# yamiel-abreu/distributed-pytorch-training

Measured on AMD Instinct MI355X. Metric: images/sec (whole node) ResNet-50 bf16 training, higher is better.
Workload: dtype bf16

## Files before the change

csrc/bindings.cpp:

```cpp
#include <ATen/ATen.h>
#include <c10/hip/HIPGuard.h>
#include <c10/hip/HIPStream.h>
#include <torch/extension.h>

#include "kernels/kernels.h"
#include "host_comm.h"
#include "pg_comm.h"
#include "rccl_comm.h"
#include "watchdog.h"
#include "reducer.h"

namespace py = pybind11;
using at::Tensor;

namespace {

hipStream_t cur_stream(const Tensor& t) {
  return c10::hip::getCurrentHIPStream(t.device().index()).stream();
}

dpt::WireType wire_of(const Tensor& t) {
  switch (t.scalar_type()) {
    case at::kFloat: return dpt::WireType::kF32;
    case at::kBFloat16: return dpt::WireType::kBF16;
// ... 1136 lines not shown
        py::arg("mask_out") = py::none());
  m.def("bn_apply", &bn_apply, py::arg("x"), py::arg("residual"), py::arg("a"), py::arg("b"), py::arg("relu"));
  m.def("bn_apply_aff", &bn_apply_aff, py::arg("x"), py::arg("x2"), py::arg("coef"), py::arg("coef2"),
        py::arg("mask_out") = py::none());
  m.def("bn2_bwd_partials", &bn2_bwd_partials, py::arg("dz"), py::arg("x"), py::arg("x2"), py::arg("weight"),
        py::arg("weight2"), py::arg("mean"), py::arg("invstd"), py::arg("mean2"), py::arg("invstd2"), py::arg("p1"),
        py::arg("p2"), py::arg("p3"), py::arg("want_dparams"));
  m.def("bn_bwd", &bn_bwd, py::arg("grad_output"), py::arg("grad_output2"), py::arg("y"), py::arg("x"),
        py::arg("weight"), py::arg("mean"), py::arg("invstd"), py::arg("relu"), py::arg("want_dz"),
        py::arg("want_dparams"), py::arg("coef") = py::none());
  m.def("ln_supported", &dpt::ln_supported, py::arg("D"));
  m.def("ln_fwd", &ln_fwd, py::arg("x"), py::arg("a"), py::arg("bias"), py::arg("gamma"), py::arg("beta"),
        py::arg("eps"), py::arg("out_kind") = 1);
  m.def("ln_bwd", &ln_bwd, py::arg("grad_s"), py::arg("grad_h"), py::arg("s"), py::arg("mean"), py::arg("rstd"),
        py::arg("gamma"), py::arg("want_ga"), py::arg("bias_like"), py::arg("want_dparams"));
  m.def("gelu_fwd", &gelu_fwd, py::arg("u"), py::arg("bias"));
  m.def("gelu_bwd", &gelu_bwd, py::arg("grad"), py::arg("u"), py::arg("bias"), py::arg("want_dbias"));
  m.def("linear_dgrad_dgelu", &linear_dgrad_dgelu, py::arg("grad"), py::arg("wt"), py::arg("u"), py::arg("bias"));
  m.def("vit_set_gelu_blocks_per_cu", &dpt::vit_set_gelu_blocks_per_cu, py::arg("n"));
  m.def("copy_rows16", &copy_rows16, py::arg("src"), py::arg("dst"));
  m.def("bias_grad16", &bias_grad16, py::arg("grad"), py::arg("out_kind"));
  m.def("sum_partials", &sum_partials, py::arg("part"), py::arg("out_kind"));
  m.def("colsum_rows", &colsum_rows, py::arg("part"), py::arg("out_kind"));
  m.def("maxpool_fwd", &maxpool_fwd, py::arg("x"), py::arg("k"), py::arg("stride"), py::arg("pad"),
        py::arg("bn_coef") = py::none());
  m.def("gap_bwd", &gap_bwd, py::arg("g"), py::arg("H"), py::arg("W"), py::arg("dtype"));
  m.def("gap_bwd_bnr", &gap_bwd_bnr, py::arg("g"), py::arg("y"), py::arg("x"), py::arg("mean"));
  m.def("maxpool_bwd", &maxpool_bwd, py::arg("grad_output"), py::arg("idx"), py::arg("H"), py::arg("W"),
        py::arg("k"), py::arg("stride"), py::arg("pad"), py::arg("grad_output2") = py::none(),
        py::arg("bn_x") = py::none(), py::arg("bn_mean") = py::none(), py::arg("bn_coef") = py::none());
  m.def("conv_fwd", &conv_fwd, py::arg("x"), py::arg("w"), py::arg("stride"), py::arg("pad"), py::arg("want_stats"),
        py::arg("out_h") = 0, py::arg("out_w") = 0);
  m.def("space_to_depth2", &space_to_depth2, py::arg("x"), py::arg("out_f16") = false);
  m.def("conv_wgrad", &conv_wgrad, py::arg("grad_output"), py::arg("x"), py::arg("weight_shape"), py::arg("stride"),
        py::arg("pad"), py::arg("fp32_out"), py::arg("target_blocks") = 0);
  m.def("conv_f32_fwd", &conv_f32_fwd, py::arg("x"), py::arg("w"), py::arg("stride"), py::arg("pad"),
        py::arg("split") = false);
  m.def("conv_f32_dgrad", &conv_f32_dgrad, py::arg("grad_output"), py::arg("w"), py::arg("stride"), py::arg("pad"),
        py::arg("H"), py::arg("W"), py::arg("split") = false);
  m.def("conv_f32_wgrad", &conv_f32_wgrad, py::arg("grad_output"), py::arg("x"), py::arg("weight_shape"),
        py::arg("stride"), py::arg("pad"), py::arg("split") = false);
  m.def("im2col", &im2col, py::arg("x"), py::arg("R"), py::arg("S"), py::arg("stride"), py::arg("pad"), py::arg("Kp"));
  m.def("attn_fwd", &attn_fwd, py::arg("qkv"), py::arg("heads"), py::arg("scale"));
  m.def("attn_set_bwd_split", &dpt::attn_set_bwd_split, py::arg("on"));
  m.def("attn_bwd", &attn_bwd, py::arg("qkv"), py::arg("out"), py::arg("grad_output"), py::arg("lse"),
        py::arg("heads"), py::arg("scale"));
  m.def("conv_set_variant", &dpt::conv_set_variant, py::arg("variant"));
  m.def("bn_set_skip_finalize", &dpt::bn_set_skip_finalize, py::arg("on"),
        "measurement only: skip every BatchNorm finalize launch (wrong values; timing upper bound)");
  m.def("conv_set_splitk_policy", &dpt::conv_set_splitk_policy, py::arg("tiles"), py::arg("eager_tiles"),
        py::arg("eager_min_k"), py::arg("target"), "split-K thresholds (A/B knob; <= 0 keeps a value)");
  m.def("conv_set_big", &dpt::conv_set_big, py::arg("on"));
  m.def("conv_set_halo", &dpt::conv_set_halo, py::arg("on"));
  m.def("conv_set_breg", &dpt::conv_set_breg, py::arg("mode"));
  m.def("conv_set_wgrad_stages", &dpt::conv_set_wgrad_stages, py::arg("mode"));
  m.def("conv_get_breg", &dpt::conv_get_breg);
  m.def("conv_set_streamk", &dpt::conv_set_streamk, py::arg("mode"), py::arg("eff") = 0.0);
  m.def("conv_get_streamk", &dpt::conv_get_streamk);
  m.def("conv_sk_prepare", &dpt::conv_sk_prepare);
  m.def("conv_sk_errors", &dpt::conv_sk_errors);
  m.def("conv_sk_blocks", &dpt::conv_sk_blocks, py::arg("tiles"), py::arg("nk"), py::arg("bn"), py::arg("mode"));
  m.def("conv_set_wgrad_target", &dpt::conv_set_wgrad_target, py::arg("blocks"));
  m.def("conv_set_wgrad_halo", &dpt::conv_set_wgrad_halo, py::arg("mode"));
  m.def("conv_fwd_splits", [](int64_t M, int Cout, int64_t K, bool graph) {
          return dpt::conv_fwd_splits_for(M, Cout, K, graph);
        }, py::arg("M"), py::arg("Cout"), py::arg("K"), py::arg("graph") = false);
  m.def("conv_set_splitk", &dpt::conv_set_splitk, py::arg("mode"));
  m.def("conv_get_splitk", &dpt::conv_get_splitk);
  m.def("conv_set_fwd_shape_policy", &dpt::conv_set_fwd_shape_policy, py::arg("bits"));
  m.def("conv_dgrad", &conv_dgrad, py::arg("grad_output"), py::arg("w"), py::arg("pad"));
  m.def("conv_dgrad_bnstats", &conv_dgrad_bnstats, py::arg("grad_output"), py::arg("w"), py::arg("pad"),
        py::arg("bn_x"), py::arg("bn_mean"), py::arg("bn_coef"), py::arg("bn_y") = py::none(),
        py::arg("bn_res") = py::none(), py::arg("w_flipped") = py::none(), py::arg("bn_x2") = py::none(),
        py::arg("bn_mean2") = py::none(), py::arg("wgrad_reduce") = nullptr, py::arg("bn_mask") = py::none());
  m.def("conv_wt_flip_multi", &conv_wt_flip_multi, py::arg("ws"));
  m.def("conv_dgrad_preflipped", &conv_dgrad_preflipped, py::arg("grad_output"), py::arg("w_flipped"), py::arg("pad"),
        py::arg("wgrad_reduce") = nullptr);
  m.def("bn_bwd_partials", &bn_bwd_partials, py::arg("grad_output"), py::arg("x"), py::arg("weight"), py::arg("mean"),
        py::arg("invstd"), py::arg("coef"), py::arg("p1"), py::arg("p2"), py::arg("want_dparams"),
        py::arg("from_dz") = false);
  m.def("conv_dgrad_s2", &conv_dgrad_s2, py::arg("grad_output"), py::arg("w"), py::arg("pad"), py::arg("H"),
        py::arg("W"), py::arg("bn_x") = py::none(), py::arg("bn_mean") = py::none(), py::arg("bn_coef") = py::none(),
        py::arg("wgrad_reduce") = nullptr);
  m.def("conv_dgrad_flip", &conv_dgrad_flip, py::arg("grad_output"), py::arg("w"), py::arg("pad"),
        py::arg("wgrad_reduce") = nullptr);
  py::class_<PendingReduce, PendingReducePtr>(m, "PendingWgradReduce")
      .def_property_readonly("done", &PendingReduce::done)
      .def_property_readonly("splits", [](const PendingReduce& p) { return p.r.splits; });
  m.def("conv_wgrad_deferred", &conv_wgrad_deferred, py::arg("grad_output"), py::arg("x"), py::arg("weight_shape"),
        py::arg("stride"), py::arg("pad"));
  m.def("conv_reduce_flush", &conv_reduce_flush, py::arg("pending"));
  m.def("rccl_version", []() { return std::string(dpt::rccl_version_string()); });

  py::class_<dpt::Collective, std::shared_ptr<dpt::Collective>>(m, "Collective")
      .def("all_reduce", [](dpt::Collective& c, Tensor t, bool on_current_stream) {
             TORCH_CHECK(t.is_cuda() && t.is_contiguous(), "all_reduce needs a contiguous GPU tensor");
             c10::hip::HIPGuard guard(t.device().index());
             hipStream_t s = cur_stream(t);
             c.all_reduce(t.data_ptr(), (size_t)t.numel(), wire_of(t), on_current_stream ? s : c.stream());
           }, py::arg("tensor"), py::arg("on_current_stream") = true)
      .def("broadcast", [](dpt::Collective& c, Tensor t, int root) {
             TORCH_CHECK(t.is_cuda() && t.is_contiguous(), "broadcast needs a contiguous GPU tensor");
             c10::hip::HIPGuard guard(t.device().index());
             c.broadcast(t.data_ptr(), (size_t)t.numel(), wire_of(t), root, cur_stream(t));
           }, py::arg("tensor"), py::arg("root") = 0)
      .def("abort", &dpt::Collective::abort)
      .def("destroy", &dpt::Collective::destroy)
      .def("check", &dpt::Collective::check)
      .def_property_readonly("kind", &dpt::Collective::kind)
      .def_property_readonly("ops", &dpt::Collective::ops)
      .def_property_readonly("sequence_hash", &dpt::Collective::sequence_hash)
      .def_property_readonly("rank", &dpt::Collective::rank)
      .def_property_readonly("world_size", &dpt::Collective::world_size)
      .def_property_readonly("device", &dpt::Collective::device)
      .def("track", [](dpt::Collective& c) {
             c10::hip::HIPGuard guard(c.device());
             c.track(c10::hip::getCurrentHIPStream(c.device()).stream());
           }, "hand the watchdog a completion marker for the work enqueued on the current stream")
      .def("_test_spin", [](dpt::Collective& c, double ms, bool on_current_stream) {
             TORCH_CHECK(ms >= 0 && ms <= 20000, "spin: 0..20000 ms");
             c10::hip::HIPGuard guard(c.device());
             dpt::launch_spin(ms, on_current_stream ? c10::hip::getCurrentHIPStream(c.device()).stream()
                                                    : c.stream());
           }, py::arg("ms"), py::arg("on_current_stream") = false,
           "test hook: enqueue a wall-clock busy-wait on the communicator (or current) stream");

  py::class_<dpt::RcclComm, dpt::Collective, std::shared_ptr<dpt::RcclComm>>(m, "RcclComm")
      .def(py::init<const std::string&, int, int, int, int, int, double>(), py::arg("unique_id"), py::arg("rank"),
           py::arg("world_size"), py::arg("device"), py::arg("min_ctas") = 0, py::arg("max_ctas") = 0,
           py::arg("init_timeout_s") = 0.0,
           py::call_guard<py::gil_scoped_release>())
      .def_property_readonly("min_ctas", &dpt::RcclComm::min_ctas)
      .def_property_readonly("max_ctas", &dpt::RcclComm::max_ctas)
      .def_property_readonly("handle", &dpt::RcclComm::handle)
      .def("inject_async_error", &dpt::RcclComm::inject_async_error, py::arg("message"))
      .def_static("new_unique_id", []() { return py::bytes(dpt::RcclComm::new_unique_id()); })
      .def("enable_watchdog", &dpt::RcclComm::enable_watchdog, py::arg("timeout_s"), py::arg("poll_s") = 0.5,
           py::arg("exit_grace_s") = 30.0)
      .def_property_readonly("watchdog_tripped", &dpt::RcclComm::watchdog_tripped)
      .def_property_readonly("watchdog_outstanding", &dpt::RcclComm::watchdog_outstanding)
      .def_property_readonly("watchdog_tracked", &dpt::RcclComm::watchdog_tracked)
      .def("async_error", &dpt::RcclComm::async_error);

  py::class_<dpt::HostBridgeComm, dpt::Collective, std::shared_ptr<dpt::HostBridgeComm>>(m, "HostBridgeComm")
      .def(py::init([](py::object ar, py::object bc, int rank, int ws, int dev, bool async_mode, py::object pg) {
             c10::intrusive_ptr<c10d::ProcessGroup> p;
             if (!pg.is_none()) p = pg.cast<c10::intrusive_ptr<c10d::ProcessGroup>>();
             return std::make_shared<dpt::HostBridgeComm>(std::move(ar), std::move(bc), rank, ws, dev, async_mode,
                                                          std::move(p));
           }),
           py::arg("all_reduce_fn"), py::arg("broadcast_fn"), py::arg("rank"), py::arg("world_size"),
           py::arg("device"), py::arg("async_mode") = false, py::arg("process_group") = py::none())
      .def_static("_process_group_size", [](py::object pg) {
             return pg.cast<c10::intrusive_ptr<c10d::ProcessGroup>>()->getSize();
           })
      .def_property_readonly("async_mode", &dpt::HostBridgeComm::async_mode)
      .def_property_readonly("completed", &dpt::HostBridgeComm::completed)
      .def("release_graph_resources", &dpt::HostBridgeComm::release_graph_resources);

  py::class_<dpt::ProcessGroupComm, dpt::Collective, std::shared_ptr<dpt::ProcessGroupComm>>(m, "ProcessGroupComm")
      .def(py::init([](py::object pg, int dev) {
             return std::make_shared<dpt::ProcessGroupComm>(pg.cast<c10::intrusive_ptr<c10d::ProcessGroup>>(), dev);
           }),
           py::arg("process_group"), py::arg("device"))
      .def_property_readonly("backend", &dpt::ProcessGroupComm::backend);

// ... 41 lines not shown
```

csrc/kernels/conv_kernels.hip:

```cpp
#include <algorithm>
#include <cmath>
#include <cstdlib>
#include <mutex>
#include <stdexcept>
#include <type_traits>

#include "carry.h"
#include "gelu.h"
#include "common.h"
#include "kernels.h"
#include "mfma.h"

namespace dpt {


#ifndef DPT_WGRAD_WAVES
#define DPT_WGRAD_WAVES 4
#endif
#ifndef DPT_CONV_HALF_EPI
#define DPT_CONV_HALF_EPI 0
#endif

namespace conv {

constexpr int BM = 128;
constexpr int BK = 64;
constexpr int kThreads = 256;
constexpr int kRowBytes = BK * 2;

__device__ __forceinline__ int swz(int row, int chunk) { return chunk ^ ((row >> 1) & 7); }

__device__ __forceinline__ int opaque_v(int v) {
  asm volatile("" : "+v"(v));
  return v;
}

__device__ __forceinline__ int xcd_remap(int bid, int nwg) {
  const int q = nwg >> 3, r = nwg & 7, xcd = bid & 7, idx = bid >> 3;
  return (xcd < r ? xcd * (q + 1) : r * (q + 1) + (xcd - r) * q) + idx;
}

}

typedef _Float16 f16x8_t __attribute__((ext_vector_type(8)));
typedef _Float16 f16x2_t __attribute__((ext_vector_type(2)));

template <bool F16>
__device__ __forceinline__ f32x16_t cmfma(bf16x8_t a, bf16x8_t b, f32x16_t c) {
  if constexpr (F16)
    return __builtin_amdgcn_mfma_f32_32x32x16_f16(__builtin_bit_cast(f16x8_t, a), __builtin_bit_cast(f16x8_t, b), c,
                                                  0, 0, 0);
  else
    return __builtin_amdgcn_mfma_f32_32x32x16_bf16(a, b, c, 0, 0, 0);
}
template <bool F16>
__device__ __forceinline__ uint32_t cpack(f32x2_t v) {
  if constexpr (F16) return __builtin_bit_cast(uint32_t, __builtin_convertvector(v, f16x2_t));
  else return __builtin_bit_cast(uint32_t, __builtin_convertvector(v, bf16x2_t));
}
template <bool F16>
__device__ __forceinline__ float cunpack(uint32_t u, int h) {
  if constexpr (F16) return (float)__builtin_bit_cast(_Float16, (uint16_t)(h ? (u >> 16) : (u & 0xffffu)));
  else return __uint_as_float(h ? (u & 0xffff0000u) : (u << 16));
}

struct ConvSk {
  float* part = nullptr;
  unsigned* flags = nullptr;
  unsigned* err = nullptr;
  int G = 0;
  uint32_t part_bytes = 0;
};

struct ConvFwdArgs {
  const uint16_t* x = nullptr;
  const uint16_t* w = nullptr;
  uint16_t* y = nullptr;
  float* psum = nullptr;
  float* psq = nullptr;
  int N = 0, H = 0, W = 0, C = 0, Ho = 0, Wo = 0, Cout = 0, R = 0, S = 0, stride = 0, pad = 0;
  int64_t M = 0;
  int m_tiles = 0, n_tiles = 0;
  int mt256 = 0;
  const uint16_t* bnx = nullptr;
  const float* bn_mean = nullptr;
  const float* bn_coef = nullptr;
  float* bp1 = nullptr;
  float* bp2 = nullptr;
  const uint16_t* bny = nullptr;
  const uint16_t* bnres = nullptr;
  const uint8_t* bnmask = nullptr;
  const uint16_t* bias16 = nullptr;
  const uint16_t* bnx2 = nullptr;
  const float* bn_mean2 = nullptr;
  float* bp3 = nullptr;
  int Rw = 0, Sw = 0, tr0 = 0, trs = 0, ts0 = 0, tss = 0;
  int oH = 0, oW = 0, oph = 0, opw = 0;
  int bp_ld = 0, bp_off = 0;
  int f16 = 0;
  float* part = nullptr;
  int splits = 1, kps = 0;
  ReduceCarry red;
  ConvSk sk;
};


template <int N>
__device__ __forceinline__ void vmcnt_wait() {
  asm volatile("s_waitcnt vmcnt(%0)" ::"n"(N) : "memory");
}

template <int RB>
__device__ __forceinline__ bf16x8_t wg_frag(const unsigned char* img, int krow0, int col0, int lane) {
  return tr_frag<RB, false>(img, krow0, col0, lane);
}

__device__ __attribute__((aligned(64))) uint4 g_conv_zero16[4];

template <int BMT, int BN, int STAGES, bool LDSEPI, bool BKN, bool STATS = true, bool BNB = false,
          bool BNR = false, bool REMAP = false, bool ZSIB = false, bool BNR2 = false, bool F16 = false,
          int NT = conv::kThreads, bool SPLIT = false, bool HALO = false, int HB = 1, bool SK = false,
          bool DGELU = false, bool BREG = false>
__global__ __launch_bounds__(NT, (SK || BREG) ? 4 : 2) void conv_fwd_kernel(ConvFwdArgs p) {
  using namespace conv;
  constexpr int BM = BMT;
  constexpr int NW = NT / 64;
  constexpr int WCOL = BREG ? 32 : 64;
  constexpr int WN = BN / WCOL;
  constexpr int WM = NW / WN;
  constexpr int MI = BM / (WM * 32);
  constexpr int NI = WCOL / 32;
  static_assert(WM * WN == NW && MI >= 1 && MI * WM * 32 == BM, "conv_fwd_kernel: bad wave tiling");
  constexpr int A_PER_T = BM * 8 / NT;
  constexpr int B_PER_T = BN * 8 / NT;
  static_assert(!HALO || (BMT == 128 && STAGES == 1 && !BKN && !SPLIT && NT == conv::kThreads), "HALO config");
  static_assert(!SK || (STAGES == 1 && !HALO && !SPLIT && LDSEPI && !BNR2 && NT == conv::kThreads), "SK config");
  static_assert(!DGELU || (BNB && !BNR && !STATS && !REMAP && LDSEPI && !SK), "DGELU config");
  static_assert(!BREG || (BMT == 128 && STAGES == 1 && LDSEPI && !BKN && !SPLIT && !SK && HB == 1 &&
                          NT == conv::kThreads && (BN == 128 || BN == 64)), "BREG config");
  constexpr int HROWS = 136;
  static_assert(HB == 1 || (HALO && HB == 3), "HB");
  constexpr int A_BYTES = (HALO ? HROWS : BM) * kRowBytes, B_BYTES = BN * kRowBytes;
  constexpr int STAGE = A_BYTES + (BREG ? 0 : HB * B_BYTES);
  constexpr int NSTAGE = BREG ? 2 : STAGES;
  constexpr int C_STRIDE = BN * 2 + 16;
  constexpr int RED = 2 * WM * BN * 4;
  constexpr int ZROW = NSTAGE * STAGE;
  constexpr int LDS_MAIN = NSTAGE * STAGE + (HALO ? kRowBytes : 0);
  constexpr bool HALF = DPT_CONV_HALF_EPI && LDSEPI && BM == 128 && NT == conv::kThreads && MI * 32 <= 64 && !BNB &&
                        !SPLIT;
  constexpr int EROWS = HALF ? 64 : BM;
  constexpr int LDS_EPI = (LDSEPI ? EROWS * C_STRIDE : 0) + RED;
  constexpr int LDS = LDS_MAIN > LDS_EPI ? LDS_MAIN : LDS_EPI;
  __shared__ __attribute__((aligned(16))) unsigned char lds[LDS];
  if constexpr (NT == conv::kThreads) {
    if (p.red.blocks) {
      const int nconv = (int)gridDim.x - p.red.blocks;
      if ((int)blockIdx.x >= nconv) {
        carry_reduce(p.red, (int)blockIdx.x - nconv, lds);
        return;
      }
    }
  }

  const int tid = threadIdx.x, lane = tid & 63, wid = tid >> 6;
  const int wm = wid / WN, wn = wid % WN;
  const int tiles = (BM == 256 ? p.mt256 : p.m_tiles) * p.n_tiles;
  const int nk_all = (int)((int64_t)p.R * p.S * p.C / BK);

  auto tile_body = [&](const int mt, const int nt, const int sp, const int ks0, const int ks1, const int sk_role,
                       const int sk_slot, const int sk_c0, const int sk_c1) {
  const int tid = SK ? conv::opaque_v((int)threadIdx.x) : (int)threadIdx.x, lane = tid & 63;
  const int wid = SK ? __builtin_amdgcn_readfirstlane(tid >> 6) : tid >> 6;
  const int wm = wid / WN, wn = wid % WN;
  const int64_t m0 = (int64_t)mt * BM;
  const int n0 = nt * BN;

  int hi0[A_PER_T], wi0[A_PER_T], aoff[A_PER_T];
  const int64_t HoWo = (int64_t)p.Ho * p.Wo;
#pragma unroll
  for (int i = 0; i < A_PER_T; ++i) {
    const int arow = (wid * A_PER_T + i) * 8 + (lane >> 3);
    const int achunk = (lane & 7) ^ ((arow >> 1) & 7);
    const int64_t m = m0 + arow;
    if (m < p.M) {
      const int64_t n = m / HoWo;
      const int rem = (int)(m - n * HoWo);
      const int ho = rem / p.Wo, wo = rem - ho * p.Wo;
      hi0[i] = ho * p.stride - p.pad;
      wi0[i] = wo * p.stride - p.pad + (p.C < BK ? achunk * 8 / p.C : 0);
      aoff[i] = (int)(((n * p.H + hi0[i]) * (int64_t)p.W + wo * p.stride - p.pad) * p.C + achunk * 8);
    } else {
      hi0[i] = -(1 << 28);
      wi0[i] = 0;
      aoff[i] = 0;
    }
  }
  const int64_t Kg = (int64_t)p.R * p.S * p.C;
  int woff[B_PER_T];
  constexpr int RBK = BN * 2;
  constexpr int KN_RPI = 1024 / RBK;
#pragma unroll
  for (int i = 0; i < B_PER_T; ++i) {
    if (BKN) {
      const int krow = (wid * B_PER_T + i) * KN_RPI + lane / (RBK / 16);
      const int kchunk = wg_slot<RBK>(krow, lane % (RBK / 16));
// ... 621 lines not shown
            *reinterpret_cast<uint4*>(p.y + m * p.Cout + n0 + oc * 8) = v;
          }
        }
      }
    }
    }
    if (BNB) {
#pragma unroll
      for (int k = 0; k < 8; ++k) {
#pragma unroll
        for (int off = CPR; off < 64; off <<= 1) {
          s1[k] += __shfl_xor(s1[k], off, 64);
          if (!DGELU) s2[k] += __shfl_xor(s2[k], off, 64);
          if (two) s3[k] += __shfl_xor(s3[k], off, 64);
        }
      }
      __syncthreads();
      constexpr int NS3 = two ? 3 : 2;
      float* bred = reinterpret_cast<float*>(lds);
      if (lane < CPR) {
#pragma unroll
        for (int k = 0; k < 8; ++k) {
          bred[(wid * NS3) * BN + oc * 8 + k] = s1[k];
          bred[(wid * NS3 + 1) * BN + oc * 8 + k] = s2[k];
          if (two) bred[(wid * NS3 + 2) * BN + oc * 8 + k] = s3[k];
        }
      }
      __syncthreads();
      if (tid < BN) {
        float a = 0.f, b = 0.f, c3 = 0.f;
#pragma unroll
        for (int w = 0; w < NW; ++w) {
          a += bred[(w * NS3) * BN + tid];
          b += bred[(w * NS3 + 1) * BN + tid];
          if (two) c3 += bred[(w * NS3 + 2) * BN + tid];
        }
        constexpr int SUBB = BM / 128;
        const int64_t pc = DGELU ? (int64_t)mt * p.Cout + n0 + tid
                                 : (int64_t)(n0 + tid) * p.bp_ld + p.bp_off + (int64_t)mt * SUBB;
        p.bp1[pc] = a;
        if (!DGELU) p.bp2[pc] = b;
        if (two) p.bp3[pc] = c3;
        if (SUBB == 2 && ((int64_t)mt * 2 + 1) * 128 < p.M) {
          p.bp1[pc + 1] = 0.f;
          if (!DGELU) p.bp2[pc + 1] = 0.f;
          if (two) p.bp3[pc + 1] = 0.f;
        }
      }
    }
  }
  };

  if constexpr (SK) {
    const uint32_t g = (uint32_t)p.sk.G >> 3, nk = (uint32_t)nk_all;
    const uint32_t x = blockIdx.x & 7, i = blockIdx.x >> 3;
    const uint32_t t_lo = (uint32_t)tiles * x / 8, t_hi = (uint32_t)tiles * (x + 1) / 8;
    const uint32_t I = (t_hi - t_lo) * nk;
    const uint32_t s0 = I * i / g, s1 = I * (i + 1) / g;
    const uint32_t f1 = min(s1, (s0 / nk + 1) * nk);
    const uint32_t nseg = s1 > s0 ? 1u + (s1 > f1 ? (s1 - 1) / nk - f1 / nk + 1 : 0u) : 0u;
    for (uint32_t q = 0; q < nseg; ++q) {
      const uint32_t b0 = q + 1 == nseg ? s0 : f1 + q * nk;
      const uint32_t tl = b0 / nk;
      const uint32_t b1 = min(s1, (tl + 1) * nk);
      const int k0 = (int)(b0 - tl * nk), k1 = (int)(b1 - tl * nk);
      int role = 0, c0 = 0, c1 = -1;
      if (k0 > 0 && k1 == nk_all) {
        role = 2;
        const uint32_t it0 = tl * nk;
        uint32_t c = it0 * g / I;
        while (c + 1 < i && I * (c + 1) / g <= it0) ++c;
        while (c > 0 && I * c / g > it0) --c;
        c0 = (int)(x + 8 * c);
        c1 = (int)blockIdx.x - 8;
      } else if (k1 < nk_all) {
        role = 1;
      }
      if (q > 0) __syncthreads();
      const int t = (int)(t_lo + tl);
      tile_body(t / p.n_tiles, t % p.n_tiles, 0, k0, k1, role, (int)blockIdx.x, c0, c1);
    }
  } else {
    const int nsplit = SPLIT ? p.splits : 1;
    const int bid0 = conv::xcd_remap(blockIdx.x, tiles * nsplit);
    const int sp = SPLIT ? bid0 % nsplit : 0;
    const int bid = SPLIT ? bid0 / nsplit : bid0;
    const int ks0 = SPLIT ? sp * p.kps : 0;
    const int ks1 = SPLIT ? min(nk_all, ks0 + p.kps) : nk_all;
    tile_body(bid / p.n_tiles, bid % p.n_tiles, sp, ks0, ks1, 0, 0, 0, -1);
  }
}

constexpr int kSplitRows = 16;
template <bool STATS, bool BNB, bool BNR, bool BNR2, bool REMAP, bool ZSIB, bool F16>
__global__ __launch_bounds__(256) void conv_split_epilogue_kernel(ConvFwdArgs p) {
  const int rb = blockIdx.x, cgb = blockIdx.y, cols = gridDim.x;
  const int tid = threadIdx.x, lane = tid & 63, wid = tid >> 6;
  const int oc = tid & 7, orow = (tid >> 3) & 15, half = tid >> 7;
  const int c0 = cgb * 64 + oc * 8;
  const int64_t MC = p.M * p.Cout;
  const int64_t m = (int64_t)rb * kSplitRows + orow;
  const bool live = m < p.M;
  const int64_t poff = (live ? m : 0) * p.Cout + c0;
  int64_t grow = live ? m : 0;
  int oy = 0, ox = 0;
  if (REMAP) {
    const int64_t hw = (int64_t)p.Ho * p.Wo, img = grow / hw, rem = grow - img * hw;
    const int a = (int)(rem / p.Wo), b = (int)(rem - (int64_t)a * p.Wo);
    oy = 2 * a + p.oph;
    ox = 2 * b + p.opw;
    grow = (img * p.oH + oy) * p.oW + ox;
  }
  const int64_t off = grow * p.Cout + c0;
  float v[8];
#pragma unroll
  for (int k = 0; k < 8; ++k) v[k] = 0.f;
  if (live) {
    for (int sp = half; sp < p.splits; sp += 2) {
      const float4* q = reinterpret_cast<const float4*>(p.part + sp * MC + poff);
      const float4 a = q[0], b = q[1];
      v[0] += a.x; v[1] += a.y; v[2] += a.z; v[3] += a.w; v[4] += b.x; v[5] += b.y; v[6] += b.z; v[7] += b.w;
    }
  }
  __shared__ float join[128][9];
  __shared__ float red[2][3][64];
  if (half == 1) {
#pragma unroll
    for (int k = 0; k < 8; ++k) join[tid & 127][k] = v[k];
  }
  __syncthreads();
  constexpr bool two = BNR && BNR2;
  float q0[8], q1[8], q2[8];
#pragma unroll
  for (int k = 0; k < 8; ++k) q0[k] = q1[k] = q2[k] = 0.f;
  if (half == 0 && live) {
#pragma unroll
    for (int k = 0; k < 8; ++k) v[k] += join[tid][k];
    uint32_t u[4];
#pragma unroll
    for (int k2 = 0; k2 < 4; ++k2) u[k2] = cpack<F16>(f32x2_t{v[2 * k2], v[2 * k2 + 1]});
    if (BNB) {
      const uint4 xv = *reinterpret_cast<const uint4*>(p.bnx + off);
      uint4 yv = make_uint4(0u, 0u, 0u, 0u), rv = yv, x2v = yv;
      uint32_t mv = 0u;
      if (BNR) {
        if (p.bnmask != nullptr) mv = p.bnmask[off >> 3];
        else yv = *reinterpret_cast<const uint4*>(p.bny + off);
        rv = *reinterpret_cast<const uint4*>(p.bnres + off);
        if (two) x2v = *reinterpret_cast<const uint4*>(p.bnx2 + off);
      }
      const uint32_t xu[4] = {xv.x, xv.y, xv.z, xv.w}, yu[4] = {yv.x, yv.y, yv.z, yv.w};
      const uint32_t ru[4] = {rv.x, rv.y, rv.z, rv.w}, x2u[4] = {x2v.x, x2v.y, x2v.z, x2v.w};
#pragma unroll
      for (int k2 = 0; k2 < 4; ++k2) {
        float dzp[2];
#pragma unroll
        for (int h = 0; h < 2; ++h) {
          const int k = 2 * k2 + h, c = c0 + k;
          const float g = cunpack<F16>(u[k2], h);
          const float x = cunpack<F16>(xu[k2], h);
          float dz;
          if (BNR) {
            const bool pos = p.bnmask != nullptr ? ((mv >> k) & 1u) != 0u : cunpack<F16>(yu[k2], h) > 0.0f;
            dz = pos ? g + cunpack<F16>(ru[k2], h) : 0.0f;
          } else {
            dz = __builtin_fmaf(x, p.bn_coef[c], p.bn_coef[p.Cout + c]) > 0.0f ? g : 0.0f;
          }
          dzp[h] = dz;
          q0[k] = dz;
          q1[k] = dz * (x - p.bn_mean[c]);
          if (two) q2[k] = dz * (cunpack<F16>(x2u[k2], h) - p.bn_mean2[c]);
        }
        if (BNR) u[k2] = cpack<F16>(f32x2_t{dzp[0], dzp[1]});
// ... 1297 lines not shown
  };
  const bool res = bny != nullptr;
  if (res && bnx2 != nullptr) run(Opts<kBnb | kBnr | kBnr2>{});
  else if (res) run(Opts<kBnb | kBnr>{});
  else run(Opts<kBnb>{});
}

void launch_linear_dgrad_dgelu(const uint16_t* dy, const uint16_t* wt, const uint16_t* u, const float* bias,
                               const uint16_t* bias16, uint16_t* gu, float* bp1, int64_t T, int n_out, int n_in,
                               bool f16, hipStream_t s) {
  if (n_in % 128 != 0 || n_out % 64 != 0) throw std::runtime_error("linear_dgrad_dgelu: n_in % 128, n_out % 64");
  ConvFwdArgs a = conv_args(dy, wt, gu, f16, 1, 1, (int)T, n_out, n_in, 1, 1, 1, 0, 1, (int)T);
  a.n_tiles = n_in / 128;
  a.bnx = u; a.bn_mean = bias; a.bias16 = bias16; a.bp1 = bp1;
  a.bp_ld = a.m_tiles;
  conv_check_offsets(a, false);
  const dim3 grid((unsigned)(a.m_tiles * a.n_tiles));
  with_bool(f16, [&](auto h) {
    launch_fwd_kernel<128, 128, 1, kLdsEpi | kBnb | kDgelu | opt(h.value, kF16)>(grid, s, a);
  });
}

int linear_dgrad_dgelu_tiles(int64_t T) { return conv_m_tiles(T); }

void launch_conv_fwd(const uint16_t* x, const uint16_t* w, uint16_t* y, int N, int H, int W, int C, int Cout,
                     int R, int S, int stride, int pad, float* psum, float* psq, hipStream_t s, int Ho, int Wo,
                     bool f16, float* ws) {
  conv_fwd_impl(x, w, y, N, H, W, C, Cout, R, S, stride, pad, psum, psq, false, s, Ho, Wo, f16, ws);
}

void launch_conv_dgrad(const uint16_t* dy, const uint16_t* w, uint16_t* dx, int N, int Ho, int Wo, int Cout, int C,
                       int R, int S, int pad, hipStream_t s, bool f16) {
  conv_fwd_impl(dy, w, dx, N, Ho, Wo, Cout, C, R, S, 1, R - 1 - pad, nullptr, nullptr, true, s, 0, 0, f16);
}

struct S2Class {
  int ph, pw, Rc, Sc, pad, Ha, Wa, tr0, ts0;
  bool zsib;
};
static int s2_classes(int H, int W, int R, int S, int pad, S2Class* out) {
  int J[2], r0[2], Js[2], s0[2], D[2];
  for (int ph = 0; ph < 2; ++ph) {
    r0[ph] = ((ph + pad) % 2 + 2) % 2;
    J[ph] = r0[ph] < R ? (R - 1 - r0[ph]) / 2 + 1 : 0;
    D[ph] = (ph + pad - r0[ph]) / 2;
    s0[ph] = r0[ph];
    Js[ph] = s0[ph] < S ? (S - 1 - s0[ph]) / 2 + 1 : 0;
  }
  const bool zsib = J[1] == 0 && Js[1] == 0 && J[0] > 0 && Js[0] > 0;
  int n = 0;
  for (int ph = 0; ph < 2; ++ph)
    for (int pw = 0; pw < 2; ++pw) {
      const int Ha = (H - ph + 1) / 2, Wa = (W - pw + 1) / 2;
      if (Ha <= 0 || Wa <= 0 || J[ph] == 0 || Js[pw] == 0) continue;
      const int pad_c = J[ph] - 1 - D[ph];
      if (Js[pw] - 1 - D[pw] != pad_c) throw std::runtime_error("conv_dgrad_s2: unequal class paddings");
      out[n++] = S2Class{ph, pw, J[ph], Js[pw], pad_c, Ha, Wa, r0[ph] + 2 * (J[ph] - 1), s0[pw] + 2 * (Js[pw] - 1),
                         zsib && ph == 0 && pw == 0};
    }
  return n;
}

ConvS2Plan conv_dgrad_s2_plan(int N, int H, int W, int C, int Cout, int R, int S, int pad, hipStream_t s) {
  S2Class cl[4];
  const int n = s2_classes(H, W, R, S, pad, cl);
  ConvS2Plan pl{0, 0};
  for (int i = 0; i < n; ++i) {
    const int64_t M = (int64_t)N * cl[i].Ha * cl[i].Wa;
    const int splits = conv_fwd_splits(M, C, (int64_t)cl[i].Rc * cl[i].Sc * Cout, nullptr, s);
    pl.chunks += splits > 1 ? conv_split_cols(M) : conv_m_tiles(M);
    if (splits > 1) pl.ws_floats = std::max(pl.ws_floats, (int64_t)splits * M * C);
  }
  return pl;
}

int conv_dgrad_s2_chunks(int N, int H, int W, int R, int S, int pad) {
  S2Class cl[4];
  const int n = s2_classes(H, W, R, S, pad, cl);
  int chunks = 0;
  for (int i = 0; i < n; ++i) chunks += conv_m_tiles((int64_t)N * cl[i].Ha * cl[i].Wa);
  return chunks;
}

void launch_conv_dgrad_s2(const uint16_t* dy, const uint16_t* w, uint16_t* dx, int N, int Ho, int Wo, int Cout,
                          int C, int R, int S, int pad, int H, int W, hipStream_t s, const uint16_t* bnx,
                          const float* bn_mean, const float* bn_coef, float* bp1, float* bp2, bool f16, float* ws) {
  const bool bnb = bnx != nullptr;
  const int bp_ld = bnb ? (ws ? conv_dgrad_s2_plan(N, H, W, C, Cout, R, S, pad, s).chunks
                              : conv_dgrad_s2_chunks(N, H, W, R, S, pad))
                        : 0;
  int bp_off = 0;
  S2Class cl[4];
  const int ncl = s2_classes(H, W, R, S, pad, cl);
  for (int ci = 0; ci < ncl; ++ci) {
    const S2Class& k = cl[ci];
    ConvFwdArgs a = conv_args(dy, w, dx, f16, N, Ho, Wo, Cout, C, k.Rc, k.Sc, 1, k.pad, k.Ha, k.Wa);
    a.Rw = R; a.Sw = S;
    a.tr0 = k.tr0; a.trs = -2;
    a.ts0 = k.ts0; a.tss = -2;
    a.oH = H; a.oW = W; a.oph = k.ph; a.opw = k.pw;
    a.bnx = bnx; a.bn_mean = bn_mean; a.bn_coef = bn_coef;
    a.bp1 = bp1; a.bp2 = bp2; a.bp_ld = bp_ld; a.bp_off = bp_off;
    if (bnb && k.zsib) throw std::runtime_error("conv_dgrad_s2: BN statistics with zero-filled classes unsupported");
    const auto run = [&](auto epi) {
      constexpr unsigned F = kBkn | kRemap | decltype(epi)::value;
      if (maybe_split<F>(a, ws, s)) {
        bp_off += conv_split_cols(a.M);
        return;
      }
      bp_off += a.m_tiles;
      fwd_launch_default<F>(a, s);
    };
    if (bnb) run(Opts<kBnb>{});
    else if (k.zsib) run(Opts<kZsib>{});
    else run(Opts<0u>{});
  }
}

static int wgrad_halo_mode(int C) {
  if (g_wgrad_halo == 5) return C == 64 ? 3 : 0;
  if (g_wgrad_halo == 6) return C == 64 ? 4 : 0;
  return g_wgrad_halo;
}

static FastDiv make_fastdiv(uint32_t d) {
  FastDiv f;
  f.d = d;
  if (d <= 1) { f.mul = 0; f.shr = 0; return f; }
  uint32_t l = 0;
  while ((1ull << l) < d) ++l;
  f.mul = (uint32_t)(((1ull << (31 + l)) + d - 1) / d);
  f.shr = l - 1;
  return f;
}

static int wgrad_target(int R, int S, int stride, int steps) {
  if (g_wgrad_target > 0) return g_wgrad_target;
  if (R * S == 1 && stride == 1) return 512;
  return steps >= 3136 ? 768 : 640;
}

ConvWgradPlan conv_wgrad_plan(int N, int H, int W, int C, int Cout, int R, int S, int stride, int pad, int Ho,
                              int Wo, int target_blocks) {
  ConvWgradPlan pl;
  pl.Ho = Ho > 0 ? Ho : (H + 2 * pad - R) / stride + 1;
  pl.Wo = Wo > 0 ? Wo : (W + 2 * pad - S) / stride + 1;
  const int64_t M = (int64_t)N * pl.Ho * pl.Wo;
  const int hmode = wgrad_halo_mode(C);
  if (hmode && R == 3 && S == 3 && stride == 1 && pad == 1 && pl.Ho == H && pl.Wo == W &&
      C % (hmode >= 3 ? 64 : 128) == 0 && Cout % 64 == 0 && (int64_t)N * H * (W + 2) + 128 < (1ll << 31)) {
    pl.halo = hmode;
    pl.bmw = 64;
    pl.bnw = pl.halo >= 3 ? 64 : 128;
    const int tiles = (Cout / 64) * 3 * (C / pl.bnw);
    const int steps = (int)(((int64_t)N * H * (W + 2) + 63) / 64);
    const int target = g_wgrad_target > 0 ? g_wgrad_target : pl.bnw == 128 ? 512 : 768;
    int splits = (target + tiles - 1) / tiles;
    const int min_steps = (int64_t)tiles * (steps / 32) >= 512 ? 32 : 2;
    splits = std::max(1, std::min(splits, steps / min_steps));
    pl.steps_per_split = (steps + splits - 1) / splits;
    pl.splits = (steps + pl.steps_per_split - 1) / pl.steps_per_split;
    pl.part_floats = pl.splits > 1 ? (int64_t)pl.splits * Cout * 9 * C : 0;
    return pl;
  }
  pl.bmw = Cout % 128 == 0 ? 128 : 64;
  pl.bnw = C % 128 == 0 ? 128 : (C == 64 && R * S > 1) ? 128 : (C == 16 && R * S * C >= 256 && pl.bmw == 64) ? 256 : 64;
  if (g_conv_variant == 20 && Cout % 256 == 0 && C % 256 == 0) pl.bmw = pl.bnw = 256;
  const int tiles = (Cout / pl.bmw) * ((R * S * C + pl.bnw - 1) / pl.bnw);
  const int steps = (int)((M + 63) / 64);
  int splits = ((target_blocks > 0 ? target_blocks : wgrad_target(R, S, stride, steps)) + tiles - 1) / tiles;
// ... 91 lines not shown
```

csrc/kernels/kernels.h:

```cpp
#pragma once

#include <hip/hip_runtime.h>
#include <stdint.h>

namespace dpt {

struct AugNorm {
  float mean[4];
  float inv_std[4];
};

void launch_grad_check(const float* g, int64_t n, const float* scale, float host_factor,
                       float* found_inf, hipStream_t s);
void launch_sgd(float* p, float* g, float* buf, int64_t n, float lr, float momentum,
                float dampening, float wd, bool nesterov, const float* scale, float host_factor,
                const float* found_inf, const float* step, bool zero_grad, uint16_t* shadow,
                int shadow_kind, hipStream_t s);
void launch_adam(float* p, float* g, float* m, float* v, int64_t n, double lr, double beta1,
                 double beta2, double eps, double wd, bool adamw, const float* scale, float host_factor,
                 const float* found_inf, const float* step, bool zero_grad, uint16_t* shadow,
                 int shadow_kind, hipStream_t s);
void launch_optim_tail(float* scale, int* growth_tracker, float* found_inf, float* step,
                       float growth_factor, float backoff_factor, int growth_interval,
                       hipStream_t s);
// ... 97 lines not shown
void conv_set_breg(int mode);
int conv_get_breg();
void conv_set_halo(int on);
void launch_linear_dgrad_dgelu(const uint16_t* dy, const uint16_t* wt, const uint16_t* u, const float* bias,
                               const uint16_t* bias16, uint16_t* gu, float* bp1, int64_t T, int n_out, int n_in,
                               bool f16, hipStream_t s);
int linear_dgrad_dgelu_tiles(int64_t T);
void conv_set_streamk(int mode, double eff);
int conv_get_streamk();
void conv_sk_prepare();
unsigned conv_sk_errors();
int conv_sk_blocks(int64_t tiles, int nk, int bn, int mode);
void conv_set_wgrad_target(int blocks);
int conv_fwd_splits(int64_t M, int Cout, int64_t K, int* kps = nullptr, hipStream_t s = nullptr);
int conv_fwd_splits_for(int64_t M, int Cout, int64_t K, bool graph, int* kps = nullptr);
int conv_split_cols(int64_t M);
void conv_set_splitk_policy(int tiles, int eager_tiles, int eager_min_k, int target);
void conv_set_splitk(int mode);
int conv_get_splitk();
void conv_set_fwd_shape_policy(int bits);
void launch_conv_fwd(const uint16_t* x, const uint16_t* w, uint16_t* y, int N, int H, int W, int C, int Cout,
                     int R, int S, int stride, int pad, float* psum, float* psq, hipStream_t s, int Ho = 0,
                     int Wo = 0, bool f16 = false, float* ws = nullptr);
struct ConvWgradPlan {
  int Ho, Wo, bmw, bnw, splits, steps_per_split;
  int64_t part_floats;
  int halo = 0;
};
void conv_set_wgrad_halo(int mode);
ConvWgradPlan conv_wgrad_plan(int N, int H, int W, int C, int Cout, int R, int S, int stride, int pad, int Ho = 0,
                              int Wo = 0, int target_blocks = 0);
struct WgradReduce {
  const float* part;
  void* out;
  int64_t n4;
  int splits, kind;
  bool consumed;
};
void launch_wgrad_reduce(const WgradReduce& r, hipStream_t s);
void launch_conv_wgrad(const uint16_t* dy, const uint16_t* x, float* part, void* dw, int dw_kind, int N, int H,
                       int W, int C, int Cout, int R, int S, int stride, int pad, const ConvWgradPlan& plan,
                       hipStream_t s, bool f16 = false, WgradReduce* defer = nullptr);
void launch_bn_bwd_apply_pre(int dtype, const void* dy, const void* x, int64_t M, int64_t C, const float* mean,
                             const float* coef, const float* kbuf, void* dx, hipStream_t s, bool from_dz);
struct ReduceCarry;
int take_attached_reduce(ReduceCarry& rc);
class AttachWgradReduce {
 public:
  AttachWgradReduce(WgradReduce* r, hipStream_t s);
  ~AttachWgradReduce();
  AttachWgradReduce(const AttachWgradReduce&) = delete;
  AttachWgradReduce& operator=(const AttachWgradReduce&) = delete;

 private:
  WgradReduce* r_;
  hipStream_t s_;
};
void launch_conv_dgrad_bnstats(const uint16_t* dy, const uint16_t* wt, uint16_t* dx, int N, int Ho, int Wo, int Cout,
                               int C, int R, int S, int pad, const uint16_t* bnx, const float* bn_mean,
                               const float* bn_coef, float* bp1, float* bp2, hipStream_t s,
                               const uint16_t* bny = nullptr, const uint16_t* bnres = nullptr,
                               const uint16_t* bnx2 = nullptr, const float* bn_mean2 = nullptr,
                               float* bp3 = nullptr, bool f16 = false, float* ws = nullptr,
                               const uint8_t* bnmask = nullptr);
constexpr int kWtFlipMax = 64;
struct WtFlipBatch {
  const uint16_t* w[kWtFlipMax];
  uint16_t* wt[kWtFlipMax];
  int Cout[kWtFlipMax], R[kWtFlipMax], S[kWtFlipMax], C[kWtFlipMax];
  int blk0[kWtFlipMax];
  int count;
};
void launch_conv_wt_flip_multi(WtFlipBatch b, hipStream_t s);
struct ConvS2Plan {
  int chunks;
  int64_t ws_floats;
};
ConvS2Plan conv_dgrad_s2_plan(int N, int H, int W, int C, int Cout, int R, int S, int pad, hipStream_t s);
void launch_conv_dgrad_s2(const uint16_t* dy, const uint16_t* w, uint16_t* dx, int N, int Ho, int Wo, int Cout,
                          int C, int R, int S, int pad, int H, int W, hipStream_t s, const uint16_t* bnx = nullptr,
                          const float* bn_mean = nullptr, const float* bn_coef = nullptr, float* bp1 = nullptr,
                          float* bp2 = nullptr, bool f16 = false, float* ws = nullptr);
int conv_dgrad_s2_chunks(int N, int H, int W, int R, int S, int pad);
void launch_conv_dgrad(const uint16_t* dy, const uint16_t* w, uint16_t* dx, int N, int Ho, int Wo, int Cout, int C,
                       int R, int S, int pad, hipStream_t s, bool f16 = false);
void launch_space_to_depth2(const void* x, bool x_bf16, uint16_t* a, int N, int H, int W, int C, hipStream_t s,
                            bool out_f16 = false);
void launch_im2col(const void* x, bool x_bf16, uint16_t* a, int N, int H, int W, int C, int R, int S, int stride,
                   int pad, int Kp, hipStream_t s);
void launch_conv_wt_flip(const uint16_t* w, uint16_t* wt, int Cout, int R, int S, int C, hipStream_t s);

bool attn_supported(int S, int Dh);
int attn_lse_stride(int S);
void attn_set_bwd_split(int on);
void launch_attn_fwd(const uint16_t* qkv, uint16_t* ctx, float* lse2, int B, int S, int H, float scale,
                     hipStream_t s);
void launch_attn_bwd(const uint16_t* qkv, const uint16_t* out, const uint16_t* dout, const float* lse2,
                     uint16_t* dqkv, int B, int S, int H, float scale, hipStream_t s);

int64_t conv_f32_workspace(int64_t M, int ncols, int K, int* splits = nullptr);
void launch_conv_f32(const float* a, const float* b, float* out, float* ws, bool dgrad, int N, int H, int W, int C,
                     int Ho, int Wo, int Co, int R, int S, int stride, int pad, hipStream_t st, bool split = false);
int64_t conv_f32_wgrad_workspace(int N, int Ho, int Wo, int Co, int J);
void launch_conv_f32_wgrad(const float* dy, const float* x, float* dw, float* ws, int N, int H, int W, int C,
                           int Ho, int Wo, int Co, int R, int S, int stride, int pad, hipStream_t st,
                           bool split = false);
}
```

Baseline: 12680.

## Launch all stride-2 dgrad parity classes as one grid

Stride-2 backward-data convolution used to issue one launch per parity class. It now builds a combined grid: classes are sorted by filter size, each class's block range is aligned to 8 for XCD remapping, and a new kernel maps each block to its class and tile. This targets launch overhead and tail underutilisation from small sequential per-class grids. It adds per-block class lookup, falls back to the old path when split-K would be used, and exposes a debug map binding.

```diff
diff --git a/csrc/bindings.cpp b/csrc/bindings.cpp
--- a/csrc/bindings.cpp
+++ b/csrc/bindings.cpp
@@ -1242,6 +1242,25 @@
   m.def("conv_dgrad_s2", &conv_dgrad_s2, py::arg("grad_output"), py::arg("w"), py::arg("pad"), py::arg("H"),
         py::arg("W"), py::arg("bn_x") = py::none(), py::arg("bn_mean") = py::none(), py::arg("bn_coef") = py::none(),
         py::arg("wgrad_reduce") = nullptr);
+  m.def("conv_set_s2_grid", &dpt::conv_set_s2_grid, py::arg("on"),
+        "stride-2 backward-data: 1 (default) the parity classes of a conv as one grid, 0 one launch per class");
+  m.def("conv_dgrad_s2_grid_map", [](int N, int H, int W, int R, int S, int pad, int n_tiles, int carry_blocks) {
+          const dpt::ConvS2Grid g = dpt::conv_dgrad_s2_grid(N, H, W, R, S, pad, n_tiles);
+          py::list classes, map;
+          for (int i = 0; i < g.n; ++i) {
+            const dpt::ConvS2Class& k = g.c[i];
+            classes.append(py::dict(py::arg("R") = k.R, py::arg("S") = k.S, py::arg("oph") = k.oph,
+                                    py::arg("opw") = k.opw, py::arg("Ho") = k.Ho, py::arg("Wo") = k.Wo,
+                                    py::arg("bp_off") = k.bp_off, py::arg("m_tiles") = k.m_tiles,
+                                    py::arg("tiles") = k.tiles, py::arg("blk0") = k.blk0));
+          }
+          for (int b = 0; b < g.blocks + carry_blocks; ++b) {
+            const dpt::ConvS2Tile t = dpt::conv_s2_block_map(g, n_tiles, carry_blocks, b);
+            map.append(py::make_tuple(t.cls, t.local, t.mt, t.nt));
+          }
+          return py::dict(py::arg("classes") = classes, py::arg("blocks") = g.blocks, py::arg("map") = map);
+        }, py::arg("N"), py::arg("H"), py::arg("W"), py::arg("R"), py::arg("S"), py::arg("pad"), py::arg("n_tiles"),
+        py::arg("carry_blocks") = 0);
   m.def("conv_dgrad_flip", &conv_dgrad_flip, py::arg("grad_output"), py::arg("w"), py::arg("pad"),
         py::arg("wgrad_reduce") = nullptr);
   py::class_<PendingReduce, PendingReducePtr>(m, "PendingWgradReduce")
diff --git a/csrc/kernels/conv_kernels.hip b/csrc/kernels/conv_kernels.hip
--- a/csrc/kernels/conv_kernels.hip
+++ b/csrc/kernels/conv_kernels.hip
@@ -17,6 +17,9 @@
 #ifndef DPT_WGRAD_WAVES
 #define DPT_WGRAD_WAVES 4
 #endif
+#ifndef DPT_S2_WAVES
+#define DPT_S2_WAVES 4
+#endif
 #ifndef DPT_CONV_HALF_EPI
 #define DPT_CONV_HALF_EPI 0
 #endif
@@ -35,7 +38,7 @@
   return v;
 }
 
-__device__ __forceinline__ int xcd_remap(int bid, int nwg) {
+__host__ __device__ __forceinline__ int xcd_remap(int bid, int nwg) {
   const int q = nwg >> 3, r = nwg & 7, xcd = bid & 7, idx = bid >> 3;
   return (xcd < r ? xcd * (q + 1) : r * (q + 1) + (xcd - r) * q) + idx;
 }
@@ -121,7 +124,7 @@
           bool BNR = false, bool REMAP = false, bool ZSIB = false, bool BNR2 = false, bool F16 = false,
           int NT = conv::kThreads, bool SPLIT = false, bool HALO = false, int HB = 1, bool SK = false,
           bool DGELU = false, bool BREG = false>
-__global__ __launch_bounds__(NT, (SK || BREG) ? 4 : 2) void conv_fwd_kernel(ConvFwdArgs p) {
+__device__ __forceinline__ void conv_fwd_body(const ConvFwdArgs& p, const int blk) {
   using namespace conv;
   constexpr int BM = BMT;
   constexpr int NW = NT / 64;
@@ -909,13 +912,58 @@
     }
   } else {
     const int nsplit = SPLIT ? p.splits : 1;
-    const int bid0 = conv::xcd_remap(blockIdx.x, tiles * nsplit);
+    const int bid0 = conv::xcd_remap(blk, tiles * nsplit);
     const int sp = SPLIT ? bid0 % nsplit : 0;
     const int bid = SPLIT ? bid0 / nsplit : bid0;
     const int ks0 = SPLIT ? sp * p.kps : 0;
     const int ks1 = SPLIT ? min(nk_all, ks0 + p.kps) : nk_all;
     tile_body(bid / p.n_tiles, bid % p.n_tiles, sp, ks0, ks1, 0, 0, 0, -1);
   }
+}
+
+template <int BMT, int BN, int STAGES, bool LDSEPI, bool BKN, bool STATS = true, bool BNB = false,
+          bool BNR = false, bool REMAP = false, bool ZSIB = false, bool BNR2 = false, bool F16 = false,
+          int NT = conv::kThreads, bool SPLIT = false, bool HALO = false, int HB = 1, bool SK = false,
+          bool DGELU = false, bool BREG = false>
+__global__ __launch_bounds__(NT, (SK || BREG) ? 4 : 2) void conv_fwd_kernel(ConvFwdArgs p) {
+  conv_fwd_body<BMT, BN, STAGES, LDSEPI, BKN, STATS, BNB, BNR, REMAP, ZSIB, BNR2, F16, NT, SPLIT, HALO, HB, SK, DGELU,
+                BREG>(p, (int)blockIdx.x);
+}
+
+__host__ __device__ inline int conv_s2_class_of(const ConvS2Grid& g, int bid, int* local) {
+  int ci = 0;
+#pragma unroll
+  for (int i = 1; i < 4; ++i)
+    if (i < g.n && bid >= g.c[i].blk0) ci = i;
+  *local = bid - g.c[ci].blk0;
+  return *local < g.c[ci].tiles ? ci : -1;
+}
+
+ConvS2Tile conv_s2_block_map(const ConvS2Grid& g, int n_tiles, int carry_blocks, int bid) {
+  ConvS2Tile t{-1, -1, -1, -1};
+  if (bid >= g.blocks && bid < g.blocks + carry_blocks) return ConvS2Tile{-2, bid - g.blocks, -1, -1};
+  if (bid < 0 || bid >= g.blocks) return t;
+  int local = 0;
+  const int ci = conv_s2_class_of(g, bid, &local);
+  if (ci < 0) return t;
+  const int tile = conv::xcd_remap(local, g.c[ci].tiles);
+  return ConvS2Tile{ci, local, tile / n_tiles, tile % n_tiles};
+}
+
+template <int BN, bool BNB, bool F16>
+__global__ __launch_bounds__(conv::kThreads, DPT_S2_WAVES) void conv_dgrad_s2_kernel(ConvFwdArgs p, ConvS2Grid g) {
+  ConvFwdArgs q = p;
+  int local = 0;
+  if ((int)blockIdx.x < g.blocks) {
+    const int ci = conv_s2_class_of(g, (int)blockIdx.x, &local);
+    if (ci < 0) return;
+    const ConvS2Class& k = g.c[ci];
+    q.R = k.R; q.S = k.S; q.pad = k.pad; q.Ho = k.Ho; q.Wo = k.Wo;
+    q.M = (int64_t)p.N * k.Ho * k.Wo;
+    q.m_tiles = k.m_tiles;
+    q.tr0 = k.tr0; q.ts0 = k.ts0; q.oph = k.oph; q.opw = k.opw; q.bp_off = k.bp_off;
+  }
+  conv_fwd_body<128, BN, 1, true, true, false, BNB, false, true, false, false, F16>(q, local);
 }
 
 constexpr int kSplitRows = 16;
@@ -2379,10 +2427,67 @@
   return chunks;
 }
 
+static int g_s2_grid = 1;
+void conv_set_s2_grid(int on) { g_s2_grid = on; }
+
+ConvS2Grid conv_dgrad_s2_grid(int N, int H, int W, int R, int S, int pad, int n_tiles, int* bp_cols) {
+  S2Class cl[4];
+  const int ncl = s2_classes(H, W, R, S, pad, cl);
+  ConvS2Grid g{};
+  g.n = ncl;
+  int bp_off = 0;
+  for (int i = 0; i < ncl; ++i) {
+    const S2Class& k = cl[i];
+    const int mt = conv_m_tiles((int64_t)N * k.Ha * k.Wa);
+    g.c[i] = ConvS2Class{k.Rc, k.Sc, k.pad, k.Ha, k.Wa, k.tr0, k.ts0, k.ph, k.pw, bp_off, mt, mt * n_tiles, 0};
+    bp_off += mt;
+  }
+  if (bp_cols) *bp_cols = bp_off;
+  std::stable_sort(g.c, g.c + ncl,
+                   [](const ConvS2Class& a, const ConvS2Class& b) { return a.R * a.S > b.R * b.S; });
+  int blk = 0;
+  for (int i = 0; i < ncl; ++i) {
+    g.c[i].blk0 = (blk + 7) & ~7;
+    blk = g.c[i].blk0 + g.c[i].tiles;
+  }
+  g.blocks = blk;
+  return g;
+}
+
 void launch_conv_dgrad_s2(const uint16_t* dy, const uint16_t* w, uint16_t* dx, int N, int Ho, int Wo, int Cout,
                           int C, int R, int S, int pad, int H, int W, hipStream_t s, const uint16_t* bnx,
                           const float* bn_mean, const float* bn_coef, float* bp1, float* bp2, bool f16, float* ws) {
   const bool bnb = bnx != nullptr;
+  if (g_s2_grid && !g_conv_sk) {
+    const int n_tiles = C % 128 == 0 ? C / 128 : C / 64;
+    int bp_cols = 0;
+    const ConvS2Grid g = conv_dgrad_s2_grid(N, H, W, R, S, pad, n_tiles, &bp_cols);
+    bool one = g.n > 1;
+    for (int i = 0; one && i < g.n; ++i)
+      one = ws == nullptr ||
+            conv_fwd_splits((int64_t)N * g.c[i].Ho * g.c[i].Wo, C, (int64_t)g.c[i].R * g.c[i].S * Cout, nullptr, s) <= 1;
+    if (one) {
+      ConvFwdArgs a = conv_args(dy, w, dx, f16, N, Ho, Wo, Cout, C, g.c[0].R, g.c[0].S, 1, g.c[0].pad, g.c[0].Ho,
+                                g.c[0].Wo);
+      a.n_tiles = n_tiles;
+      a.Rw = R; a.Sw = S;
+      a.trs = -2; a.tss = -2;
+      a.oH = H; a.oW = W;
+      a.bnx = bnx; a.bn_mean = bn_mean; a.bn_coef = bn_coef;
+      a.bp1 = bp1; a.bp2 = bp2; a.bp_ld = bnb ? bp_cols : 0;
+      conv_check_offsets(a, true);
+      const dim3 grid((unsigned)(g.blocks + take_attached_reduce(a.red)));
+      with_bool(C % 128 == 0, [&](auto wide) {
+        with_bool(bnb, [&](auto b) {
+          with_bool(f16, [&](auto h) {
+            hipLaunchKernelGGL((conv_dgrad_s2_kernel<wide.value ? 128 : 64, b.value, h.value>), grid,
+                               dim3(conv::kThreads), 0, s, a, g);
+          });
+        });
+      });
+      return;
+    }
+  }
   const int bp_ld = bnb ? (ws ? conv_dgrad_s2_plan(N, H, W, C, Cout, R, S, pad, s).chunks
                               : conv_dgrad_s2_chunks(N, H, W, R, S, pad))
                         : 0;
diff --git a/csrc/kernels/kernels.h b/csrc/kernels/kernels.h
--- a/csrc/kernels/kernels.h
+++ b/csrc/kernels/kernels.h
@@ -203,6 +203,24 @@
                           const float* bn_mean = nullptr, const float* bn_coef = nullptr, float* bp1 = nullptr,
                           float* bp2 = nullptr, bool f16 = false, float* ws = nullptr);
 int conv_dgrad_s2_chunks(int N, int H, int W, int R, int S, int pad);
+struct ConvS2Class {
+  int R, S, pad, Ho, Wo, tr0, ts0, oph, opw;
+  int bp_off;
+  int m_tiles;
+  int tiles;
+  int blk0;
+};
+struct ConvS2Grid {
+  int n;
+  int blocks;
+  ConvS2Class c[4];
+};
+void conv_set_s2_grid(int on);
+ConvS2Grid conv_dgrad_s2_grid(int N, int H, int W, int R, int S, int pad, int n_tiles, int* bp_cols = nullptr);
+struct ConvS2Tile {
+  int cls, local, mt, nt;
+};
+ConvS2Tile conv_s2_block_map(const ConvS2Grid& g, int n_tiles, int carry_blocks, int bid);
 void launch_conv_dgrad(const uint16_t* dy, const uint16_t* w, uint16_t* dx, int N, int Ho, int Wo, int Cout, int C,
                        int R, int S, int pad, hipStream_t s, bool f16 = false);
 void launch_space_to_depth2(const void* x, bool x_bf16, uint16_t* a, int N, int H, int W, int C, hipStream_t s,
```

New measurement: 12800, median of 6. No clear change (+1.0%).
